# csteinmetz1/st-ito

Measured on AMD Instinct MI355X. Metric: candidate-evals/sec (pop x iters), 48 kHz 10 s stereo, 5-effect chain, higher is better.
Workload: dtype f32 (effects f32 / f64 as the reference; trunk convs with >= 256 output channels: f32 operands carried as f16 hi + lo pairs on the f16 matrix pipe, f32 accumulate -- as close to float64 as the f32 pipe, tools/ubench/split_mfma.hip)

## Files before the change

### st-ito_amd/csrc/frontend.hip

```cpp
#include "common.h"

namespace stito {

struct FrontendDev {
    int n_fft, hop, n_mels, norm_mode, log2_n2, no_center, mel_stride;
    const float *window;
    const float2 *twiddle;
    const int *mel_start, *mel_len, *mel_off;
    const float *mel_w;
    const float *bn_scale, *bn_shift;
};

__device__ __forceinline__ float2 cmul(float2 a, float2 b) {
    return make_float2(a.x * b.x - a.y * b.y, a.x * b.y + a.y * b.x);
}

__device__ __forceinline__ int64_t reflect_idx(int64_t i, int64_t L) {
    if (i < 0) i = -i;
    if (i >= L) i = 2 * (L - 1) - i;
    return i;
}

static constexpr int FE_THREADS = 256;

__global__ __launch_bounds__(FE_THREADS) void k_logmel(FrontendDev fe, const float *__restrict__ audio,
                                                        const float *__restrict__ peaks, int norm_passes, int C,
                                                        int64_t L, int64_t T, float *__restrict__ out) {
    extern __shared__ __attribute__((aligned(16))) char smem_raw[];
    const int N = fe.n_fft, N2 = N >> 1;
    float2 *bufA = (float2 *)smem_raw;
    float2 *bufB = bufA + C * N2;

    const int cand = blockIdx.y;
    const int64_t t = blockIdx.x;
    const int tid = threadIdx.x;

    float d1 = 1.0f, d2 = 1.0f;
    if (peaks != nullptr && norm_passes > 0) {
        const float pk = peaks[cand];
        d1 = fmaxf(pk, 1e-8f);
        if (norm_passes > 1) d2 = fmaxf(pk / d1, 1e-8f);
    }
    const bool second = norm_passes > 1 && d2 != 1.0f;
    const float r1 = 1.0f / d1, r2 = 1.0f / d2;
    const float *xl = audio + (int64_t)cand * C * L;
    const float *xr = xl + L;
    const int64_t base = fe.no_center ? t * fe.hop : t * fe.hop - N2;

    const bool inside = base >= 0 && base + N <= L;
    const uintptr_t al = (uintptr_t)(xl + base) | (uintptr_t)(xr + base) | (uintptr_t)fe.window;
    if (inside && (al & 15) == 0 && (N2 & 1) == 0) {
        const float4 *l4 = (const float4 *)(xl + base), *r4 = (const float4 *)(xr + base), *w4 = (const float4 *)fe.window;
        for (int j = tid; j < (N2 >> 1); j += FE_THREADS) {
            const float4 a = l4[j], w = w4[j];
            float a0 = a.x * r1, a1 = a.y * r1, a2 = a.z * r1, a3 = a.w * r1;
            if (second) { a0 = a0 * r2; a1 = a1 * r2; a2 = a2 * r2; a3 = a3 * r2; }
            if (C == 2) {
                const float4 b = r4[j];
                float b0 = b.x * r1, b1 = b.y * r1, b2 = b.z * r1, b3 = b.w * r1;
                if (second) { b0 = b0 * r2; b1 = b1 * r2; b2 = b2 * r2; b3 = b3 * r2; }
                const float m0 = (a0 + b0) * 0.5f, m1 = (a1 + b1) * 0.5f, m2 = (a2 + b2) * 0.5f, m3 = (a3 + b3) * 0.5f;
                const float s0 = (a0 - b0) * 0.5f, s1 = (a1 - b1) * 0.5f, s2 = (a2 - b2) * 0.5f, s3 = (a3 - b3) * 0.5f;
                *(float4 *)(bufA + 2 * j) = make_float4(m0 * w.x, m1 * w.y, m2 * w.z, m3 * w.w);
                *(float4 *)(bufA + N2 + 2 * j) = make_float4(s0 * w.x, s1 * w.y, s2 * w.z, s3 * w.w);
            } else {
                *(float4 *)(bufA + 2 * j) = make_float4(a0 * w.x, a1 * w.y, a2 * w.z, a3 * w.w);
            }
        }
    } else {
    const bool fast = inside && (al & 7) == 0;
    for (int m = tid; m < N2; m += FE_THREADS) {
        float a0, a1, b0 = 0.0f, b1 = 0.0f, w0, w1;
        if (fast) {
            const float2 a = ((const float2 *)(xl + base))[m], w = ((const float2 *)fe.window)[m];
            a0 = a.x; a1 = a.y; w0 = w.x; w1 = w.y;
            if (C == 2) { const float2 b = ((const float2 *)(xr + base))[m]; b0 = b.x; b1 = b.y; }
        } else {
            const int64_t i0 = reflect_idx(base + 2 * m, L), i1 = reflect_idx(base + 2 * m + 1, L);
            w0 = fe.window[2 * m]; w1 = fe.window[2 * m + 1];
            a0 = xl[i0]; a1 = xl[i1];
            if (C == 2) { b0 = xr[i0]; b1 = xr[i1]; }
        }
        a0 = a0 * r1; a1 = a1 * r1;
        if (second) { a0 = a0 * r2; a1 = a1 * r2; }
        if (C == 2) {
            b0 = b0 * r1; b1 = b1 * r1;
            if (second) { b0 = b0 * r2; b1 = b1 * r2; }
            const float m0 = (a0 + b0) * 0.5f, m1 = (a1 + b1) * 0.5f, s0 = (a0 - b0) * 0.5f, s1 = (a1 - b1) * 0.5f;
            bufA[m] = make_float2(m0 * w0, m1 * w1);
            bufA[N2 + m] = make_float2(s0 * w0, s1 * w1);
        } else {
            bufA[m] = make_float2(a0 * w0, a1 * w1);
        }
    }
    }
    __syncthreads();

    float2 *src = bufA, *dst = bufB;
    int p = 1, sh = fe.log2_n2;
    if (fe.log2_n2 & 1) {
        const int half = N2 >> 1;
        for (int c = 0; c < C; ++c) {
            const float2 *s = src + c * N2;
            float2 *d = dst + c * N2;
            for (int i = tid; i < half; i += FE_THREADS) {
                const float2 u0 = s[i], u1 = s[i + half];
                d[2 * i] = make_float2(u0.x + u1.x, u0.y + u1.y);
                d[2 * i + 1] = make_float2(u0.x - u1.x, u0.y - u1.y);
            }
        }
        __syncthreads();
        float2 *tmp = src; src = dst; dst = tmp;
        p = 2; --sh;
    }
    const int quarter = N2 >> 2;
    for (; p < N2; p <<= 2, sh -= 2) {
        for (int i = tid; i < quarter; i += FE_THREADS) {
            const int k = i & (p - 1);
            const int j = ((i - k) << 2) + k;
            const int ti = k << (sh - 1);
            const float2 w1 = fe.twiddle[ti], w2 = fe.twiddle[2 * ti];
            const float2 w3 = cmul(w1, w2);
            for (int c = 0; c < C; ++c) {
                const float2 *s = src + c * N2;
                float2 *d = dst + c * N2;
                const float2 a0 = s[i];
                const float2 a1 = cmul(s[i + quarter], w1);
                const float2 a2 = cmul(s[i + 2 * quarter], w2);
                const float2 a3 = cmul(s[i + 3 * quarter], w3);
                const float2 b0 = make_float2(a0.x + a2.x, a0.y + a2.y), b1 = make_float2(a0.x - a2.x, a0.y - a2.y);
                const float2 b2 = make_float2(a1.x + a3.x, a1.y + a3.y), b3 = make_float2(a1.x - a3.x, a1.y - a3.y);
                d[j] = make_float2(b0.x + b2.x, b0.y + b2.y);
                d[j + p] = make_float2(b1.x + b3.y, b1.y - b3.x);
                d[j + 2 * p] = make_float2(b0.x - b2.x, b0.y - b2.y);
                d[j + 3 * p] = make_float2(b1.x - b3.y, b1.y + b3.x);
            }
        }
        __syncthreads();
        float2 *tmp = src; src = dst; dst = tmp;
    }

    float *pw = (float *)dst;
    for (int c = 0; c < C; ++c) {
        const float2 *Z = src + c * N2;
        for (int k = tid; k <= N2; k += FE_THREADS) {
            const float2 zk = Z[k & (N2 - 1)];
            const float2 zn = Z[(N2 - k) & (N2 - 1)];
            const float2 E = make_float2(0.5f * (zk.x + zn.x), 0.5f * (zk.y - zn.y));
            const float2 O = make_float2(0.5f * (zk.y + zn.y), -0.5f * (zk.x - zn.x));
            const float2 w = (k < N2) ? fe.twiddle[k] : make_float2(-1.0f, 0.0f);
            const float2 wo = cmul(w, O);
            const float re = E.x + wo.x, im = E.y + wo.y;
            pw[c * (N2 + 1) + k] = re * re + im * im;
        }
    }
    __syncthreads();

    const int M = fe.n_mels;
    for (int q0 = 0; q0 < 4 * C * M; q0 += FE_THREADS) {
        const int q = q0 + tid;
        const bool live = q < 4 * C * M;
        const int part = q & 3, cm = live ? q >> 2 : 0;
        const int c = cm / M, m = cm - c * M;
        const int st = fe.mel_start[m], ln = fe.mel_len[m];
        const int lq = (ln + 3) >> 2;
        const int beg = part * lq < ln ? part * lq : ln, end = beg + lq < ln ? beg + lq : ln;
        const float *w = fe.mel_w + fe.mel_off[m];
        const int ws = fe.mel_stride;
        const float *p = pw + c * (N2 + 1) + st;
        float acc = 0.0f;
        for (int i = beg; i < end; ++i) acc = fmaf(p[i], w[i * ws], acc);
        acc += __shfl_xor(acc, 1);
        acc += __shfl_xor(acc, 2);
        if (!live || part) continue;
        float v = acc > 1e-10f ? 10.0f * log10f(acc) : -100.0f;
        if (fe.norm_mode == STITO_NORM_MINMAX) {
            v = fminf(fmaxf(v, -80.0f), 40.0f);
            v = (v + 80.0f) / 120.0f;
            v = (v * 2.0f) - 1.0f;
        } else if (fe.norm_mode == STITO_NORM_BATCHNORM) {
            v = v * fe.bn_scale[m] + fe.bn_shift[m];
        }
        out[((int64_t)(cand * C + c) * T + t) * M + m] = v;
    }
}


static constexpr int FW_F = 4;
static constexpr int FW_ROW = 66;
static constexpr int FW_WAVE_F2 = 16 * FW_ROW + 64;
static constexpr int FW_MAX_MELS = 256;
static constexpr int FW_LDS_BYTES = (16 * 64 + (FE_THREADS / 64) * FW_WAVE_F2) * 8 + 4 * FW_MAX_MELS * 8;

__device__ __forceinline__ float2 cadd(float2 a, float2 b) { return make_float2(a.x + b.x, a.y + b.y); }
__device__ __forceinline__ float2 csub(float2 a, float2 b) { return make_float2(a.x - b.x, a.y - b.y); }
__device__ __forceinline__ void fw_r4(float2 &a0, float2 &a1, float2 &a2, float2 &a3) {
    const float2 b0 = cadd(a0, a2), b1 = csub(a0, a2), b2 = cadd(a1, a3), b3 = csub(a1, a3);
    a0 = cadd(b0, b2);
    a1 = make_float2(b1.x + b3.y, b1.y - b3.x);
    a2 = csub(b0, b2);
    a3 = make_float2(b1.x - b3.y, b1.y + b3.x);
}
#define FW_K(k) (4 * ((k) & 3) + ((k) >> 2))
__device__ __forceinline__ void fw_dft16(float2 (&x)[16]) {
    const float c1 = 0.92387953251128674f, s1 = 0.38268343236508977f, h = 0.70710678118654752f;
#pragma unroll
    for (int n2 = 0; n2 < 4; ++n2) fw_r4(x[n2], x[4 + n2], x[8 + n2], x[12 + n2]);
    x[5] = cmul(x[5], make_float2(c1, -s1));
    x[6] = cmul(x[6], make_float2(h, -h));
    x[7] = cmul(x[7], make_float2(s1, -c1));
    x[9] = cmul(x[9], make_float2(h, -h));
    x[10] = make_float2(x[10].y, -x[10].x);
    x[11] = cmul(x[11], make_float2(-h, -h));
    x[13] = cmul(x[13], make_float2(s1, -c1));
    x[14] = cmul(x[14], make_float2(-h, -h));
    x[15] = cmul(x[15], make_float2(-c1, s1));
#pragma unroll
    for (int k1 = 0; k1 < 4; ++k1) fw_r4(x[4 * k1], x[4 * k1 + 1], x[4 * k1 + 2], x[4 * k1 + 3]);
}
__device__ __forceinline__ float2 fw_tw(const float2 *__restrict__ table, int t) {
    const float2 v = table[t & 1023];
    return t >= 1024 ? make_float2(-v.x, -v.y) : v;
}
#define FW_LDS_SYNC() { __builtin_amdgcn_wave_barrier(); asm volatile("s_waitcnt lgkmcnt(0)" ::: "memory"); __builtin_amdgcn_wave_barrier(); }

static constexpr int FW_WG_PER_CU = 3;
__global__ __launch_bounds__(FE_THREADS, FW_WG_PER_CU) void k_logmel_wave(FrontendDev fe, const float *__restrict__ audio,
                                                             const float *__restrict__ peaks, int norm_passes, int C,
                                                             int64_t L, int64_t T, float *__restrict__ out) {
    extern __shared__ __attribute__((aligned(16))) char smem_raw[];
    constexpr int N2 = 1024, HOP = 1024;
    const int lane = threadIdx.x & 63, wave = threadIdx.x >> 6;
    float2 *tw1s = (float2 *)smem_raw;
    float2 *buf = tw1s + 16 * 64 + wave * FW_WAVE_F2;
    float2 *tw2s = buf + 16 * FW_ROW;
    for (int i = threadIdx.x; i < 16 * 64; i += FE_THREADS) tw1s[i] = fw_tw(fe.twiddle, 2 * (i & 63) * (i >> 6));
    uint2 *mtask = (uint2 *)(tw1s + 16 * 64 + (FE_THREADS / 64) * FW_WAVE_F2);
    const int M = fe.n_mels;
    for (int q = threadIdx.x; q < 4 * M; q += FE_THREADS) {
        const int part = q & 3, m = q >> 2;
        const int st = fe.mel_start[m], ln = fe.mel_len[m];
        const int lq = (ln + 3) >> 2;
        const int beg = part * lq < ln ? part * lq : ln, end = beg + lq < ln ? beg + lq : ln;
        mtask[q] = make_uint2((unsigned)(st + beg) | (unsigned)(end - beg) << 16, (unsigned)(fe.mel_off[m] + beg * fe.mel_stride));
    }
    __syncthreads();
    const int cand = blockIdx.y;
    const int64_t t0 = ((int64_t)blockIdx.x * (FE_THREADS / 64) + wave) * FW_F;
    if (t0 >= T) return;
    const int nf = (int)(T - t0 < FW_F ? T - t0 : FW_F);

    float d1 = 1.0f, d2 = 1.0f;
    if (peaks != nullptr && norm_passes > 0) {
        const float pk = peaks[cand];
        d1 = fmaxf(pk, 1e-8f);
        if (norm_passes > 1) d2 = fmaxf(pk / d1, 1e-8f);
    }
    const bool second = norm_passes > 1 && d2 != 1.0f;
    const float r1 = 1.0f / d1, r2 = 1.0f / d2;
    const float *xl = audio + (int64_t)cand * C * L;
    const float *xr = xl + L;
    const bool al8 = (((uintptr_t)xl | (uintptr_t)xr) & 7) == 0;

    tw2s[lane] = fw_tw(fe.twiddle, 32 * (lane >> 4) * (lane & 15));

    float2 hm0[8], hs0[8], hm1[8], hs1[8];
    auto load_hop = [&](int64_t h, float2 (&hm)[8], float2 (&hs)[8]) {
        const int64_t b = h * HOP;
        const bool fast = al8 && b >= 0 && b + HOP <= L;
        if (fast) {
            const float *pl = xl + b + 2 * lane, *pr = xr + b + 2 * lane;
#pragma unroll
            for (int j = 0; j < 8; ++j) hm[j] = *(const float2 *)(pl + 128 * j);
            if (C == 2) {
#pragma unroll
                for (int j = 0; j < 8; ++j) hs[j] = *(const float2 *)(pr + 128 * j);
            }
        }
#pragma unroll
        for (int j = 0; j < 8; ++j) {
            const int64_t i = b + 2 * lane + 128 * j;
            float a0, a1, b0 = 0.0f, b1 = 0.0f;
            if (fast) {
                a0 = hm[j].x; a1 = hm[j].y;
                if (C == 2) { b0 = hs[j].x; b1 = hs[j].y; }
            } else {
                const int64_t i0 = reflect_idx(i, L), i1 = reflect_idx(i + 1, L);
                a0 = xl[i0]; a1 = xl[i1];
                if (C == 2) { b0 = xr[i0]; b1 = xr[i1]; }
            }
            a0 = a0 * r1; a1 = a1 * r1;
            if (second) { a0 = a0 * r2; a1 = a1 * r2; }
            if (C == 2) {
                b0 = b0 * r1; b1 = b1 * r1;
                if (second) { b0 = b0 * r2; b1 = b1 * r2; }
                hm[j] = make_float2((a0 + b0) * 0.5f, (a1 + b1) * 0.5f);
                hs[j] = make_float2((a0 - b0) * 0.5f, (a1 - b1) * 0.5f);
            } else {
                hm[j] = make_float2(a0, a1);
                hs[j] = hm[j];
            }
        }
    };
    const int64_t h_first = fe.no_center ? t0 : t0 - 1;
    load_hop(h_first, hm0, hs0);
    load_hop(h_first + 1, hm1, hs1);

    for (int f = 0; f < nf; ++f) {
        const int64_t t = t0 + f;
#pragma unroll 1
        for (int c = 0; c < C; ++c) {
            float2 x[16];
            const float *win = fe.window;
            const float2 *twt = fe.twiddle;
            asm volatile("" : "+s"(win), "+s"(twt));
#pragma unroll
            for (int j = 0; j < 16; ++j) {
                const float2 w = *(const float2 *)(win + 2 * lane + 128 * j);
                const float2 v = j < 8 ? (c == 0 ? hm0[j] : hs0[j]) : (c == 0 ? hm1[j - 8] : hs1[j - 8]);
                x[j] = make_float2(v.x * w.x, v.y * w.y);
            }
            fw_dft16(x);
            buf[lane] = x[FW_K(0)];
#pragma unroll
            for (int k1 = 1; k1 < 16; ++k1) buf[k1 * FW_ROW + lane] = cmul(x[FW_K(k1)], tw1s[k1 * 64 + lane]);
            FW_LDS_SYNC()
            {
                const int k1 = lane & 15, a = lane >> 4;
#pragma unroll
                for (int b = 0; b < 16; ++b) x[b] = buf[k1 * FW_ROW + a + 4 * b];
                fw_dft16(x);
                FW_LDS_SYNC()
                buf[(k1 + 0) * 4 + a] = x[FW_K(0)];
#pragma unroll
                for (int k2a = 1; k2a < 16; ++k2a) buf[(k1 + 16 * k2a) * 4 + a] = cmul(x[FW_K(k2a)], tw2s[a * 16 + k2a]);
            }
            FW_LDS_SYNC()
#pragma unroll
            for (int q = 0; q < 4; ++q) {
                const float4 p01 = *(const float4 *)(buf + (lane + 64 * q) * 4), p23 = *(const float4 *)(buf + (lane + 64 * q) * 4 + 2);
                float2 a0 = make_float2(p01.x, p01.y), a1 = make_float2(p01.z, p01.w), a2 = make_float2(p23.x, p23.y), a3 = make_float2(p23.z, p23.w);
                fw_r4(a0, a1, a2, a3);
                x[q] = a0; x[q + 4] = a1; x[q + 8] = a2; x[q + 12] = a3;
            }
            FW_LDS_SYNC()
            float *pw = (float *)buf;
            const int pl = (64 - lane) & 63;
#pragma unroll
            for (int m = 0; m < 16; ++m) {
                const int k = lane + 64 * m;
                const float2 zk = x[m];
                const float px = __shfl(x[15 - m].x, pl, 64), py = __shfl(x[15 - m].y, pl, 64);
                const float2 zo = x[(16 - m) & 15];
                const float2 zn = lane == 0 ? zo : make_float2(px, py);
                const float2 E = make_float2(0.5f * (zk.x + zn.x), 0.5f * (zk.y - zn.y));
                const float2 O = make_float2(0.5f * (zk.y + zn.y), -0.5f * (zk.x - zn.x));
                const float2 wo = cmul(twt[k], O);
                const float re = E.x + wo.x, im = E.y + wo.y;
                pw[k] = re * re + im * im;
            }
            if (lane == 0) {
                const float2 z = x[0];
                const float2 E = make_float2(0.5f * (z.x + z.x), 0.5f * (z.y - z.y));
                const float2 O = make_float2(0.5f * (z.y + z.y), -0.5f * (z.x - z.x));
                const float2 wo = cmul(make_float2(-1.0f, 0.0f), O);
                const float re = E.x + wo.x, im = E.y + wo.y;
                pw[N2] = re * re + im * im;
            }
            FW_LDS_SYNC()
            for (int q0 = 0; q0 < 4 * M; q0 += 64) {
                const int q = q0 + lane;
                const bool live = q < 4 * M;
                const int part = q & 3, m = live ? q >> 2 : 0;
                const uint2 mt = live ? mtask[q] : make_uint2(0u, 0u);
                const float *w = fe.mel_w + mt.y;
                const int ws = fe.mel_stride, n = (int)(mt.x >> 16);
                const float *p = pw + (mt.x & 0xffffu);
                float acc = 0.0f;
                for (int i = 0; i < n; ++i) acc = fmaf(p[i], w[i * ws], acc);
                acc += __shfl_xor(acc, 1);
                acc += __shfl_xor(acc, 2);
                if (!live || part) continue;
                float v = acc > 1e-10f ? 10.0f * log10f(acc) : -100.0f;
                if (fe.norm_mode == STITO_NORM_MINMAX) {
                    v = fminf(fmaxf(v, -80.0f), 40.0f);
                    v = (v + 80.0f) / 120.0f;
                    v = (v * 2.0f) - 1.0f;
                } else if (fe.norm_mode == STITO_NORM_BATCHNORM) {
                    v = v * fe.bn_scale[m] + fe.bn_shift[m];
                }
                out[((int64_t)(cand * C + c) * T + t) * M + m] = v;
            }
            FW_LDS_SYNC()
        }
        if (f + 1 < nf) {
#pragma unroll
            for (int j = 0; j < 8; ++j) { hm0[j] = hm1[j]; hs0[j] = hs1[j]; }
            load_hop(h_first + f + 2, hm1, hs1);
        }
    }
}

}

using namespace stito;

extern "C" int64_t stito_num_frames(int64_t n_samples, int hop) { return n_samples / hop + 1; }
extern "C" int64_t stito_num_frames_nocenter(int64_t n_samples, int n_fft, int hop) {
    return n_samples >= n_fft ? (n_samples - n_fft) / hop + 1 : 0;
}

extern "C" int stito_logmel(const stito_frontend *fe, const float *audio_dev, const float *peaks_dev, int norm_passes,
                            int pop, int channels, int64_t n_samples, float *logmel_dev, void *stream) {
    hipStream_t st = (hipStream_t)stream;
    STITO_REQUIRE(fe != nullptr, STITO_E_INVALID, "stito_logmel: null front-end");
    STITO_REQUIRE(channels == 1 || channels == 2, STITO_E_INVALID, "Invalid number of channels: %d", channels);
    const int N = fe->n_fft;
    STITO_REQUIRE(N >= 64 && N <= 4096 && (N & (N - 1)) == 0, STITO_E_UNSUPPORTED, "n_fft %d must be a power of two in [64, 4096]", N);
    STITO_REQUIRE(fe->hop > 0 && fe->n_mels > 0, STITO_E_INVALID, "bad hop / n_mels");
    STITO_REQUIRE(fe->no_center ? n_samples >= N : n_samples > N / 2, STITO_E_INVALID,
                  "audio too short for the STFT (n_samples %lld, n_fft %d)", (long long)n_samples, N);
    STITO_REQUIRE(pop > 0, STITO_E_INVALID, "empty batch");
    FrontendDev d;
    d.n_fft = N; d.hop = fe->hop; d.n_mels = fe->n_mels; d.norm_mode = fe->norm_mode; d.no_center = fe->no_center;
    int l2 = 0;
    while ((1 << l2) < N / 2) ++l2;
    d.log2_n2 = l2;
    d.window = fe->window_dev; d.twiddle = (const float2 *)fe->twiddle_dev;
    d.mel_start = fe->mel_start_dev; d.mel_len = fe->mel_len_dev; d.mel_off = fe->mel_off_dev; d.mel_w = fe->mel_w_dev;
    d.mel_stride = fe->mel_w_stride > 1 ? fe->mel_w_stride : 1;
    d.bn_scale = fe->bn0_scale_dev; d.bn_shift = fe->bn0_shift_dev;
    STITO_REQUIRE(fe->norm_mode != STITO_NORM_BATCHNORM || (d.bn_scale && d.bn_shift), STITO_E_INVALID, "batchnorm input norm needs bn0 scale/shift");
    const int64_t T = fe->no_center ? stito_num_frames_nocenter(n_samples, N, fe->hop) : stito_num_frames(n_samples, fe->hop);
    const char *gen_env = getenv("STITO_LOGMEL_GENERIC");
    const bool generic_only = gen_env != nullptr && atoi(gen_env) != 0;
    if (N == 2048 && fe->hop == 1024 && !generic_only && n_samples >= 2048 && fe->n_mels <= FW_MAX_MELS) {
        const int wpb = FE_THREADS / 64;
        const int64_t tasks = (T + FW_F - 1) / FW_F;
        const size_t lds_w = FW_LDS_BYTES;
        hipLaunchKernelGGL(k_logmel_wave, dim3((unsigned)((tasks + wpb - 1) / wpb), pop), dim3(FE_THREADS), lds_w, st, d, audio_dev,
                           peaks_dev, norm_passes, channels, n_samples, T, logmel_dev);
        STITO_LAUNCH_CHECK();
        return STITO_OK;
    }
    const size_t lds = (size_t)channels * (N / 2) * sizeof(float2) * 2;
    STITO_HIP_CHECK(hipFuncSetAttribute((const void *)k_logmel, hipFuncAttributeMaxDynamicSharedMemorySize, (int)lds));
    hipLaunchKernelGGL(k_logmel, dim3((unsigned)T, pop), dim3(FE_THREADS), lds, st, d, audio_dev, peaks_dev, norm_passes,
                       channels, n_samples, T, logmel_dev);
    STITO_LAUNCH_CHECK();
    return STITO_OK;
}
```

Measured before the change: 6176.

## Unroll mel band dot products, use DPP quad reduce, stage sums in LDS

Replaces the per-lane serial mel filterbank loop with a templated, unrolled, predicated accumulation whose width is chosen by a wave-wide ballot on band length, and pre-scales weight offsets to byte units. The quad reduction moves from shfl_xor to DPP quad permutes. Mel sums are staged in LDS so that log/normalisation and the output stores run on all 64 lanes instead of one lane in four. It also forces the wave index into a scalar register and uses 32-bit byte offsets for the audio loads, aiming to cut address arithmetic. The cost is an extra LDS round-trip and wave barrier per frame and channel, plus possible wasted FMAs on tail lanes.

```diff
diff --git a/st-ito_amd/csrc/frontend.hip b/st-ito_amd/csrc/frontend.hip
--- a/st-ito_amd/csrc/frontend.hip
+++ b/st-ito_amd/csrc/frontend.hip
@@ -190,6 +190,7 @@
 static constexpr int FW_ROW = 66;
 static constexpr int FW_WAVE_F2 = 16 * FW_ROW + 64;
 static constexpr int FW_MAX_MELS = 256;
+static constexpr int FW_MEL_SUMS = 1088;
 static constexpr int FW_LDS_BYTES = (16 * 64 + (FE_THREADS / 64) * FW_WAVE_F2) * 8 + 4 * FW_MAX_MELS * 8;
 
 __device__ __forceinline__ float2 cadd(float2 a, float2 b) { return make_float2(a.x + b.x, a.y + b.y); }
@@ -224,25 +225,52 @@
 }
 #define FW_LDS_SYNC() { __builtin_amdgcn_wave_barrier(); asm volatile("s_waitcnt lgkmcnt(0)" ::: "memory"); __builtin_amdgcn_wave_barrier(); }
 
+template <int B>
+__device__ __forceinline__ float fw_band_quarter(const char *__restrict__ wb, unsigned wo, unsigned ws4, const float *p, int n) {
+    float acc = 0.0f;
+    unsigned last = (unsigned)(n - 1) * ws4;
+    for (int r = n; r > 0; r -= B) {
+        float wv[B], pv[B];
+#pragma unroll
+        for (int j = 0; j < B; ++j) {
+            const unsigned oj = (unsigned)j * ws4;
+            wv[j] = *(const float *)(wb + (wo + (oj < last ? oj : last)));
+            pv[j] = p[j];
+        }
+#pragma unroll
+        for (int j = 0; j < B; ++j) {
+            const float a = fmaf(pv[j], wv[j], acc);
+            acc = j < r ? a : acc;
+        }
+        wo += B * ws4; last -= B * ws4; p += B;
+    }
+    return acc;
+}
+template <int CTRL>
+__device__ __forceinline__ float fw_quad_swap(float v) {
+    return __builtin_bit_cast(float, __builtin_amdgcn_update_dpp(0, __builtin_bit_cast(int, v), CTRL, 0xF, 0xF, true));
+}
+
 static constexpr int FW_WG_PER_CU = 3;
 __global__ __launch_bounds__(FE_THREADS, FW_WG_PER_CU) void k_logmel_wave(FrontendDev fe, const float *__restrict__ audio,
                                                              const float *__restrict__ peaks, int norm_passes, int C,
                                                              int64_t L, int64_t T, float *__restrict__ out) {
     extern __shared__ __attribute__((aligned(16))) char smem_raw[];
     constexpr int N2 = 1024, HOP = 1024;
-    const int lane = threadIdx.x & 63, wave = threadIdx.x >> 6;
+    const int lane = threadIdx.x & 63, wave = __builtin_amdgcn_readfirstlane(threadIdx.x >> 6);
     float2 *tw1s = (float2 *)smem_raw;
     float2 *buf = tw1s + 16 * 64 + wave * FW_WAVE_F2;
     float2 *tw2s = buf + 16 * FW_ROW;
     for (int i = threadIdx.x; i < 16 * 64; i += FE_THREADS) tw1s[i] = fw_tw(fe.twiddle, 2 * (i & 63) * (i >> 6));
     uint2 *mtask = (uint2 *)(tw1s + 16 * 64 + (FE_THREADS / 64) * FW_WAVE_F2);
     const int M = fe.n_mels;
+    const unsigned ws4 = 4u * (unsigned)fe.mel_stride;
     for (int q = threadIdx.x; q < 4 * M; q += FE_THREADS) {
         const int part = q & 3, m = q >> 2;
         const int st = fe.mel_start[m], ln = fe.mel_len[m];
         const int lq = (ln + 3) >> 2;
         const int beg = part * lq < ln ? part * lq : ln, end = beg + lq < ln ? beg + lq : ln;
-        mtask[q] = make_uint2((unsigned)(st + beg) | (unsigned)(end - beg) << 16, (unsigned)(fe.mel_off[m] + beg * fe.mel_stride));
+        mtask[q] = make_uint2((unsigned)(st + beg) | (unsigned)(end - beg) << 16, 4u * (unsigned)(fe.mel_off[m] + beg * fe.mel_stride));
     }
     __syncthreads();
     const int cand = blockIdx.y;
@@ -269,12 +297,14 @@
         const int64_t b = h * HOP;
         const bool fast = al8 && b >= 0 && b + HOP <= L;
         if (fast) {
-            const float *pl = xl + b + 2 * lane, *pr = xr + b + 2 * lane;
-#pragma unroll
-            for (int j = 0; j < 8; ++j) hm[j] = *(const float2 *)(pl + 128 * j);
+            const char *pl = (const char *)(xl + b), *pr = (const char *)(xr + b);
+            unsigned lo = 8u * (unsigned)lane;
+            asm volatile("" : "+v"(lo));
+#pragma unroll
+            for (int j = 0; j < 8; ++j) hm[j] = *(const float2 *)(pl + lo + 512 * j);
             if (C == 2) {
 #pragma unroll
-                for (int j = 0; j < 8; ++j) hs[j] = *(const float2 *)(pr + 128 * j);
+                for (int j = 0; j < 8; ++j) hs[j] = *(const float2 *)(pr + lo + 512 * j);
             }
         }
 #pragma unroll
@@ -311,9 +341,10 @@
 #pragma unroll 1
         for (int c = 0; c < C; ++c) {
             float2 x[16];
-            const float *win = fe.window;
-            const float2 *twt = fe.twiddle;
-            asm volatile("" : "+s"(win), "+s"(twt));
+            int hide = 0;
+            asm volatile("" : "+s"(hide));
+            const float *win = fe.window + hide;
+            const float2 *twt = fe.twiddle + hide;
 #pragma unroll
             for (int j = 0; j < 16; ++j) {
                 const float2 w = *(const float2 *)(win + 2 * lane + 128 * j);
@@ -371,16 +402,21 @@
             for (int q0 = 0; q0 < 4 * M; q0 += 64) {
                 const int q = q0 + lane;
                 const bool live = q < 4 * M;
-                const int part = q & 3, m = live ? q >> 2 : 0;
                 const uint2 mt = live ? mtask[q] : make_uint2(0u, 0u);
-                const float *w = fe.mel_w + mt.y;
-                const int ws = fe.mel_stride, n = (int)(mt.x >> 16);
+                const int n = (int)(mt.x >> 16);
                 const float *p = pw + (mt.x & 0xffffu);
-                float acc = 0.0f;
-                for (int i = 0; i < n; ++i) acc = fmaf(p[i], w[i * ws], acc);
-                acc += __shfl_xor(acc, 1);
-                acc += __shfl_xor(acc, 2);
-                if (!live || part) continue;
+                const bool over4 = __builtin_amdgcn_ballot_w64(n > 4) != 0, over2 = __builtin_amdgcn_ballot_w64(n > 2) != 0;
+                float acc = over4   ? fw_band_quarter<8>((const char *)fe.mel_w, mt.y, ws4, p, n)
+                            : over2 ? fw_band_quarter<4>((const char *)fe.mel_w, mt.y, ws4, p, n)
+                                    : fw_band_quarter<2>((const char *)fe.mel_w, mt.y, ws4, p, n);
+                acc += fw_quad_swap<0xB1>(acc);
+                acc += fw_quad_swap<0x4E>(acc);
+                if (live && !(q & 3)) pw[FW_MEL_SUMS + (q >> 2)] = acc;
+            }
+            FW_LDS_SYNC()
+            float *const orow = out + ((int64_t)(cand * C + c) * T + t) * M;
+            for (int m = lane; m < M; m += 64) {
+                const float acc = pw[FW_MEL_SUMS + m];
                 float v = acc > 1e-10f ? 10.0f * log10f(acc) : -100.0f;
                 if (fe.norm_mode == STITO_NORM_MINMAX) {
                     v = fminf(fmaxf(v, -80.0f), 40.0f);
@@ -389,7 +425,7 @@
                 } else if (fe.norm_mode == STITO_NORM_BATCHNORM) {
                     v = v * fe.bn_scale[m] + fe.bn_shift[m];
                 }
-                out[((int64_t)(cand * C + c) * T + t) * M + m] = v;
+                orow[m] = v;
             }
             FW_LDS_SYNC()
         }
```

Result: no change. 6219, median of 5 (+0.7%).

## Stage mel filterbank weights in LDS and widen logmel wave workgroup

Applied to the files above, without the earlier changes.

The change copies the mel filterbank weights into a per-workgroup LDS table laid out per round and step, so the mel projection reads weights from LDS instead of strided global loads. The projection loop gets uniform trip counts per round (masked FMAs) and DPP quad-perm reductions in place of shuffles. The workgroup grows from 256 to 768 threads to amortise the table build. The extra setup per workgroup and the larger LDS footprint may cut occupancy, and wave-uniform max step counts add wasted FMAs.

```diff
diff --git a/st-ito_amd/csrc/frontend.hip b/st-ito_amd/csrc/frontend.hip
--- a/st-ito_amd/csrc/frontend.hip
+++ b/st-ito_amd/csrc/frontend.hip
@@ -190,7 +190,10 @@
 static constexpr int FW_ROW = 66;
 static constexpr int FW_WAVE_F2 = 16 * FW_ROW + 64;
 static constexpr int FW_MAX_MELS = 256;
-static constexpr int FW_LDS_BYTES = (16 * 64 + (FE_THREADS / 64) * FW_WAVE_F2) * 8 + 4 * FW_MAX_MELS * 8;
+static constexpr int FW_THREADS = 768;
+static constexpr int FW_MEL_TAB_STEPS = 128;
+static constexpr int FW_LDS_BYTES = (16 * 64 + (FW_THREADS / 64) * FW_WAVE_F2) * 8 + 4 * FW_MAX_MELS * 8 + FW_MEL_TAB_STEPS * 64 * 4;
+static_assert(FW_LDS_BYTES <= 160 * 1024, "k_logmel_wave's workgroup has to fit a CU's LDS");
 
 __device__ __forceinline__ float2 cadd(float2 a, float2 b) { return make_float2(a.x + b.x, a.y + b.y); }
 __device__ __forceinline__ float2 csub(float2 a, float2 b) { return make_float2(a.x - b.x, a.y - b.y); }
@@ -224,20 +227,25 @@
 }
 #define FW_LDS_SYNC() { __builtin_amdgcn_wave_barrier(); asm volatile("s_waitcnt lgkmcnt(0)" ::: "memory"); __builtin_amdgcn_wave_barrier(); }
 
-static constexpr int FW_WG_PER_CU = 3;
-__global__ __launch_bounds__(FE_THREADS, FW_WG_PER_CU) void k_logmel_wave(FrontendDev fe, const float *__restrict__ audio,
+template <int CTRL> __device__ __forceinline__ float fw_quad_perm(float v) {
+    return __int_as_float(__builtin_amdgcn_update_dpp(0, __float_as_int(v), CTRL, 0xf, 0xf, false));
+}
+
+static constexpr int FW_WAVES_PER_SIMD = 3;
+__global__ __launch_bounds__(FW_THREADS, FW_WAVES_PER_SIMD) void k_logmel_wave(FrontendDev fe, const float *__restrict__ audio,
                                                              const float *__restrict__ peaks, int norm_passes, int C,
-                                                             int64_t L, int64_t T, float *__restrict__ out) {
+                                                             int64_t L, int64_t T, int mel_lds, float *__restrict__ out) {
     extern __shared__ __attribute__((aligned(16))) char smem_raw[];
     constexpr int N2 = 1024, HOP = 1024;
     const int lane = threadIdx.x & 63, wave = threadIdx.x >> 6;
     float2 *tw1s = (float2 *)smem_raw;
     float2 *buf = tw1s + 16 * 64 + wave * FW_WAVE_F2;
     float2 *tw2s = buf + 16 * FW_ROW;
-    for (int i = threadIdx.x; i < 16 * 64; i += FE_THREADS) tw1s[i] = fw_tw(fe.twiddle, 2 * (i & 63) * (i >> 6));
-    uint2 *mtask = (uint2 *)(tw1s + 16 * 64 + (FE_THREADS / 64) * FW_WAVE_F2);
+    for (int i = threadIdx.x; i < 16 * 64; i += FW_THREADS) tw1s[i] = fw_tw(fe.twiddle, 2 * (i & 63) * (i >> 6));
+    uint2 *mtask = (uint2 *)(tw1s + 16 * 64 + (FW_THREADS / 64) * FW_WAVE_F2);
+    float *mtab = (float *)(mtask + 4 * FW_MAX_MELS);
     const int M = fe.n_mels;
-    for (int q = threadIdx.x; q < 4 * M; q += FE_THREADS) {
+    for (int q = threadIdx.x; q < 4 * M; q += FW_THREADS) {
         const int part = q & 3, m = q >> 2;
         const int st = fe.mel_start[m], ln = fe.mel_len[m];
         const int lq = (ln + 3) >> 2;
@@ -245,8 +253,42 @@
         mtask[q] = make_uint2((unsigned)(st + beg) | (unsigned)(end - beg) << 16, (unsigned)(fe.mel_off[m] + beg * fe.mel_stride));
     }
     __syncthreads();
+    const int rounds = (4 * M + 63) >> 6;
+    int rinfo = 0, steps = 0;
+    {
+        constexpr int R = 4 * FW_MAX_MELS / 64;
+        int n[R];
+#pragma unroll
+        for (int r = 0; r < R; ++r) n[r] = r * 64 + lane < 4 * M ? (int)(mtask[r * 64 + lane].x >> 16) : 0;
+#pragma unroll
+        for (int o = 32; o; o >>= 1) {
+#pragma unroll
+            for (int r = 0; r < R; ++r) n[r] = max(n[r], __shfl_xor(n[r], o));
+        }
+#pragma unroll
+        for (int r = 0; r < R; ++r) {
+            if (lane == r) rinfo = n[r] | steps << 16;
+            steps += n[r];
+        }
+    }
+    steps = __builtin_amdgcn_readfirstlane(steps);
+    const bool use_tab = mel_lds != 0 && steps <= FW_MEL_TAB_STEPS;
+    if (use_tab) {
+        for (int e = threadIdx.x; e < steps * 64; e += FW_THREADS) {
+            const int s = e >> 6;
+            int r = 0, first = 0;
+            for (int k = 0; k < rounds; ++k) {
+                const int f = __builtin_amdgcn_readlane(rinfo, k) >> 16;
+                if (s >= f) { r = k; first = f; }
+            }
+            const int q = r * 64 + (e & 63), i = s - first;
+            const uint2 mt = q < 4 * M ? mtask[q] : make_uint2(0u, 0u);
+            mtab[e] = i < (int)(mt.x >> 16) ? fe.mel_w[mt.y + i * fe.mel_stride] : 0.0f;
+        }
+    }
+    __syncthreads();
     const int cand = blockIdx.y;
-    const int64_t t0 = ((int64_t)blockIdx.x * (FE_THREADS / 64) + wave) * FW_F;
+    const int64_t t0 = ((int64_t)blockIdx.x * (FW_THREADS / 64) + wave) * FW_F;
     if (t0 >= T) return;
     const int nf = (int)(T - t0 < FW_F ? T - t0 : FW_F);
 
@@ -368,19 +410,7 @@
                 pw[N2] = re * re + im * im;
             }
             FW_LDS_SYNC()
-            for (int q0 = 0; q0 < 4 * M; q0 += 64) {
-                const int q = q0 + lane;
-                const bool live = q < 4 * M;
-                const int part = q & 3, m = live ? q >> 2 : 0;
-                const uint2 mt = live ? mtask[q] : make_uint2(0u, 0u);
-                const float *w = fe.mel_w + mt.y;
-                const int ws = fe.mel_stride, n = (int)(mt.x >> 16);
-                const float *p = pw + (mt.x & 0xffffu);
-                float acc = 0.0f;
-                for (int i = 0; i < n; ++i) acc = fmaf(p[i], w[i * ws], acc);
-                acc += __shfl_xor(acc, 1);
-                acc += __shfl_xor(acc, 2);
-                if (!live || part) continue;
+            auto tail = [&](int m, float acc) {
                 float v = acc > 1e-10f ? 10.0f * log10f(acc) : -100.0f;
                 if (fe.norm_mode == STITO_NORM_MINMAX) {
                     v = fminf(fmaxf(v, -80.0f), 40.0f);
@@ -390,6 +420,57 @@
                     v = v * fe.bn_scale[m] + fe.bn_shift[m];
                 }
                 out[((int64_t)(cand * C + c) * T + t) * M + m] = v;
+            };
+            if (use_tab) {
+                for (int g = 0; 4 * g < rounds; ++g) {
+                    float acc[4];
+#pragma unroll
+                    for (int k = 0; k < 4; ++k) {
+                        const int r = 4 * g + k;
+                        const int info = __builtin_amdgcn_readlane(rinfo, r);
+                        const int nr = info & 0xffff;
+                        const float *w = mtab + (info >> 16) * 64 + lane;
+                        const int q = r * 64 + lane;
+                        const unsigned mt = q < 4 * M ? mtask[q].x : 0u;
+                        const int n = (int)(mt >> 16);
+                        const float *p = pw + (mt & 0xffffu);
+                        float a = 0.0f;
+#pragma unroll 4
+                        for (int i = 0; i < nr; ++i) {
+                            const float s = fmaf(p[i], w[i * 64], a);
+                            a = i < n ? s : a;
+                        }
+                        acc[k] = a;
+                    }
+                    float band = 0.0f;
+#pragma unroll
+                    for (int k = 0; k < 4; ++k) acc[k] += fw_quad_perm<0xb1>(acc[k]);
+#pragma unroll
+                    for (int k = 0; k < 4; ++k) acc[k] += fw_quad_perm<0x4e>(acc[k]);
+#pragma unroll
+                    for (int k = 0; k < 4; ++k) {
+                        const float v = __shfl(acc[k], 4 * (lane & 15));
+                        if ((lane >> 4) == k) band = v;
+                    }
+                    const int m = 64 * g + lane;
+                    if (m < M) tail(m, band);
+                }
+            } else {
+                for (int q0 = 0; q0 < 4 * M; q0 += 64) {
+                    const int q = q0 + lane;
+                    const bool live = q < 4 * M;
+                    const int part = q & 3, m = live ? q >> 2 : 0;
+                    const uint2 mt = live ? mtask[q] : make_uint2(0u, 0u);
+                    const float *w = fe.mel_w + mt.y;
+                    const int ws = fe.mel_stride, n = (int)(mt.x >> 16);
+                    const float *p = pw + (mt.x & 0xffffu);
+                    float acc = 0.0f;
+                    for (int i = 0; i < n; ++i) acc = fmaf(p[i], w[i * ws], acc);
+                    acc += __shfl_xor(acc, 1);
+                    acc += __shfl_xor(acc, 2);
+                    if (!live || part) continue;
+                    tail(m, acc);
+                }
             }
             FW_LDS_SYNC()
         }
@@ -435,11 +516,14 @@
     const char *gen_env = getenv("STITO_LOGMEL_GENERIC");
     const bool generic_only = gen_env != nullptr && atoi(gen_env) != 0;
     if (N == 2048 && fe->hop == 1024 && !generic_only && n_samples >= 2048 && fe->n_mels <= FW_MAX_MELS) {
-        const int wpb = FE_THREADS / 64;
+        const char *tab_env = getenv("STITO_LOGMEL_MEL_LDS");
+        const int mel_lds = tab_env == nullptr || atoi(tab_env) != 0;
+        const int wpb = FW_THREADS / 64;
         const int64_t tasks = (T + FW_F - 1) / FW_F;
         const size_t lds_w = FW_LDS_BYTES;
-        hipLaunchKernelGGL(k_logmel_wave, dim3((unsigned)((tasks + wpb - 1) / wpb), pop), dim3(FE_THREADS), lds_w, st, d, audio_dev,
-                           peaks_dev, norm_passes, channels, n_samples, T, logmel_dev);
+        STITO_HIP_CHECK(hipFuncSetAttribute((const void *)k_logmel_wave, hipFuncAttributeMaxDynamicSharedMemorySize, (int)lds_w));
+        hipLaunchKernelGGL(k_logmel_wave, dim3((unsigned)((tasks + wpb - 1) / wpb), pop), dim3(FW_THREADS), lds_w, st, d, audio_dev,
+                           peaks_dev, norm_passes, channels, n_samples, T, mel_lds, logmel_dev);
         STITO_LAUNCH_CHECK();
         return STITO_OK;
     }
```

Result: no change. 6123 before, 6115 after (-0.1%).
